# nvpro-samples/vk_gltf_renderer

Measured on AMD Instinct MI355X. Metric: Msamples/s (and ms/frame @ fixed spp) 1080p & 4K, 1/2/4/8 MI355X, higher is better.
Workload: dtype f32

## Files before the change

vk_gltf_renderer_amd/csrc/device/mi_pt_api.hip:

```cpp
#include <hip/hip_runtime.h>

#include <algorithm>
#include <chrono>
#include <cstdlib>
#include <cmath>
#include <cstdio>
#include <cstring>
#include <memory>
#include <string>
#include <vector>

#include "mi_pt.h"
#include "bvh_refit.h"
#include "material_patch.h"
#include "pt_build.h"
#include "pt_bvh.h"
#include "pt_deform.h"
#include "pt_kernels.h"

namespace {

thread_local std::string g_lastError;

int fail(int code, const std::string& msg)
// ... 248 lines not shown
  hipStream_t             lastStream = nullptr;
  hipStream_t             sideStream = nullptr;
  hipEvent_t              evShaded = nullptr, evShadowed = nullptr;

  ~MiPt()
  {
    if(bvhNodes)
      (void)hipFree(bvhNodes);
    if(bvhTris)
      (void)hipFree(bvhTris);
    if(bvh8Nodes)
      (void)hipFree(bvh8Nodes);
    for(hipEvent_t e : eventPool)
      (void)hipEventDestroy(e);
    for(hipEvent_t e : fcDone)
      if(e)
        (void)hipEventDestroy(e);
    if(fcHost)
      (void)hipHostFree(fcHost);
    if(sideStream)
      (void)hipStreamDestroy(sideStream);
    if(evShaded)
      (void)hipEventDestroy(evShaded);
    if(evShadowed)
      (void)hipEventDestroy(evShadowed);
  }
};

namespace {

size_t align16(size_t v) { return (v + 15u) & ~size_t(15); }

int allocPathResources(MiPt* pt, int frames)
{
  if(size_t(pt->numSlots) * size_t(frames) >= 0x7fffffffull)
    return fail(MI_PT_ERR_ARGUMENT, "too many path slots: reduce the frames in flight or the resolution");
  pt->framesCap          = frames;
  const size_t n         = std::max(size_t(pt->numSlots) * size_t(frames), size_t(1));
  HIP_TRY(pt->pathArrays.alloc(n));
  HIP_TRY(pt->firstHit.alloc(std::max(size_t(pt->numSlots), size_t(1))));
  pt->haveFirstHit = false;
  pt->optThroughput.release(); pt->optMisc.release(); pt->optMedium.release(); pt->optPixelSum.release(); pt->optGuides.release(); pt->optShadowAux2.release();
  pt::PathSoA& P = pt->paths;
  P              = pt::PathSoA{};
  P.radiance     = pt->pathArrays.ptr;
  P.firstHit     = pt->firstHit.ptr;
  const size_t numChunks = (n + pt::QCHUNK - 1) / pt::QCHUNK;
  const size_t subCap    = ((numChunks + pt::NSUB - 1) / pt::NSUB + 1) * pt::QCHUNK;
  const size_t qsize     = subCap * pt::NSUB;
  if(qsize >= (size_t(1) << 31))
    return fail(MI_PT_ERR_ARGUMENT, "mi_pt_render_frames: " + std::to_string(frames) + " frames in flight x " + std::to_string(pt->numSlots)
                                        + " pixel slots exceed 2^31 path slots");
  HIP_TRY(pt->queueMem.alloc(qsize * 3 + pt::QC_COUNT));
  HIP_TRY(pt->queuePayload.alloc(qsize * 14));
  pt->queueCap = qsize;
  pt::RayQueue* qs[3] = {&pt->queues.active[0], &pt->queues.active[1], &pt->queues.shadow};
  for(int i = 0; i < 3; ++i)
    qs[i]->slot = pt->queueMem.ptr + qsize * size_t(i);
  for(int i = 0; i < 2; ++i)
  {
    qs[i]->org  = pt->queuePayload.ptr + qsize * size_t(5 * i + 0);
    qs[i]->dir  = pt->queuePayload.ptr + qsize * size_t(5 * i + 1);
    qs[i]->aux2 = pt->queuePayload.ptr + qsize * size_t(5 * i + 2);
    qs[i]->misc = pt->queuePayload.ptr + qsize * size_t(5 * i + 3);
    qs[i]->rad  = pt->queuePayload.ptr + qsize * size_t(5 * i + 4);
    qs[i]->aux  = pt->queuePayload.ptr + qsize * 10;
  }
  pt->queues.shadow.org  = pt->queuePayload.ptr + qsize * 11;
  pt->queues.shadow.dir  = pt->queuePayload.ptr + qsize * 12;
  pt->queues.shadow.aux  = pt->queuePayload.ptr + qsize * 13;
  pt->queues.shadow.aux2 = nullptr;
  pt->queues.shadow.misc = pt->queues.shadow.rad = nullptr;
  pt->queues.counters = pt->queueMem.ptr + 3 * qsize;
  pt->queues.subCap   = uint32_t(subCap);
  pt->queues.candPool = nullptr; pt->queues.candNext = nullptr; pt->queues.overflow = nullptr;
  pt->queues.candCap  = 0;
  size_t candCap = qsize * 2;
  if(pt->sw.candPoolSet)
    candCap = pt->sw.candPool;
  if(pt->hasTransmissive && pt->wide && candCap > 0)
  {
    candCap = std::min(candCap, size_t(0x7fffffff));
    HIP_TRY(pt->candPool.alloc(candCap));
    HIP_TRY(pt->candLists.alloc(candCap + qsize));
    pt->queues.candPool = pt->candPool.ptr;
    pt->queues.candNext = pt->candLists.ptr;
    pt->queues.overflow = pt->candLists.ptr + candCap;
    pt->queues.candCap  = uint32_t(candCap);
  }
  HIP_TRY(hipMemset(pt->queues.counters, 0, sizeof(uint32_t) * pt::QC_COUNT));
  return MI_PT_OK;
}

int ensureOptionalPathArrays(MiPt* pt, bool stateBySlot, bool multiSample, bool guides, bool catcher)
{
  const size_t n = std::max(size_t(pt->numSlots) * size_t(pt->framesCap), size_t(1));
  auto need = [&](DevBuf<float4>& b, size_t count) -> int {
    if(b.ptr)
      return MI_PT_OK;
    HIP_TRY(hipDeviceSynchronize());
    HIP_TRY(b.alloc(count));
    HIP_TRY(hipMemset(b.ptr, 0, count * sizeof(float4)));
    return MI_PT_OK;
  };
  pt::PathSoA& P = pt->paths;
  if(stateBySlot || multiSample)
  {
    if(int rc = need(pt->optMisc, n)) return rc;
    P.misc = pt->optMisc.ptr;
  }
  if(stateBySlot)
  {
    if(int rc = need(pt->optThroughput, n)) return rc;
    P.throughput = pt->optThroughput.ptr;
  }
  if(multiSample)
  {
    if(int rc = need(pt->optPixelSum, n)) return rc;
    P.pixelSum = pt->optPixelSum.ptr;
  }
  if(!pt->simpleMaterials)
  {
    if(int rc = need(pt->optMedium, n)) return rc;
// ... 2020 lines not shown
```

vk_gltf_renderer_amd/csrc/device/pt_bvh.h:

```cpp
#pragma once
#include "pt_scene.h"

namespace pt {

#ifndef MI_BVH8_STACK_LDS
#define MI_BVH8_STACK_LDS 12
#endif
constexpr int BVH_STACK_LDS  = 2 * MI_BVH8_STACK_LDS;
constexpr int BVH_STACK_PRIV = 72;
constexpr int BVH_EMPTY      = int(0x80000000u);

struct TriHit
{
  float t, u, v;
  bool  front;
};

PT_DEV bool intersectTri(f3 v0, f3 e1, f3 e2, f3 org, f3 dir, TriHit& h)
{
#pragma clang fp contract(off)
  f3    pvec = crossFma(dir, e2);
  float det  = dotFma(e1, pvec);
  if(det == 0.0f)
    return false;
  float inv  = divExact(1.0f, det);
  f3    tvec = org - v0;
  float u    = dotFma(tvec, pvec) * inv;
  if(u < 0.0f || u > 1.0f)
    return false;
  f3    qvec = crossFma(tvec, e1);
  float v    = dotFma(dir, qvec) * inv;
  if(v < 0.0f || u + v > 1.0f)
    return false;
  h.t     = dotFma(e2, qvec) * inv;
  h.u     = u;
  h.v     = v;
  h.front = det > 0.0f;
  return true;
}

struct RaySetup
{
  f3 org, dir, idir, ood;
};
PT_DEV RaySetup makeRaySetup(f3 org, f3 dir)
{
  RaySetup    r;
  const float eps = 1e-30f;
  r.org           = org;
  r.dir           = dir;
  r.idir.x        = divExact(1.0f, fabsf(dir.x) < eps ? copysignf(eps, dir.x) : dir.x);
  r.idir.y        = divExact(1.0f, fabsf(dir.y) < eps ? copysignf(eps, dir.y) : dir.y);
  r.idir.z        = divExact(1.0f, fabsf(dir.z) < eps ? copysignf(eps, dir.z) : dir.z);
  r.ood           = org * r.idir;
  return r;
}

struct LaneStack
{
  int* lds;
  int  tid;
  int  stride;
  int* priv;
  int  sp;
  PT_DEV void push(int v)
  {
    if(sp < BVH_STACK_LDS)
      lds[sp * stride + tid] = v;
    else if(sp - BVH_STACK_LDS < BVH_STACK_PRIV)
      priv[sp - BVH_STACK_LDS] = v;
    ++sp;
  }
  PT_DEV int pop()
  {
    --sp;
    if(sp < BVH_STACK_LDS)
      return lds[sp * stride + tid];
    if(sp - BVH_STACK_LDS < BVH_STACK_PRIV)
      return priv[sp - BVH_STACK_LDS];
    return BVH_EMPTY;
  }
};

PT_DEV int bvhInnerStep(const DevScene& sc, const RaySetup& r, float tmax, int cur, LaneStack& st)
{
  const float4* n  = sc.bvhNodes + size_t(cur) * 4;
  const float4  n0 = n[0], n1 = n[1], n2 = n[2], n3 = n[3];
  float c0x0 = __fmaf_rn(n0.x, r.idir.x, -r.ood.x), c0x1 = __fmaf_rn(n0.y, r.idir.x, -r.ood.x);
  float c0y0 = __fmaf_rn(n0.z, r.idir.y, -r.ood.y), c0y1 = __fmaf_rn(n0.w, r.idir.y, -r.ood.y);
  float c0z0 = __fmaf_rn(n2.x, r.idir.z, -r.ood.z), c0z1 = __fmaf_rn(n2.y, r.idir.z, -r.ood.z);
  float c1x0 = __fmaf_rn(n1.x, r.idir.x, -r.ood.x), c1x1 = __fmaf_rn(n1.y, r.idir.x, -r.ood.x);
  float c1y0 = __fmaf_rn(n1.z, r.idir.y, -r.ood.y), c1y1 = __fmaf_rn(n1.w, r.idir.y, -r.ood.y);
  float c1z0 = __fmaf_rn(n2.z, r.idir.z, -r.ood.z), c1z1 = __fmaf_rn(n2.w, r.idir.z, -r.ood.z);
  float t0n  = fmaxf(fmaxf(fminf(c0x0, c0x1), fminf(c0y0, c0y1)), fmaxf(fminf(c0z0, c0z1), 0.0f));
  float t0f  = fminf(fminf(fmaxf(c0x0, c0x1), fmaxf(c0y0, c0y1)), fminf(fmaxf(c0z0, c0z1), tmax));
  float t1n  = fmaxf(fmaxf(fminf(c1x0, c1x1), fminf(c1y0, c1y1)), fmaxf(fminf(c1z0, c1z1), 0.0f));
  float t1f  = fminf(fminf(fmaxf(c1x0, c1x1), fmaxf(c1y0, c1y1)), fminf(fmaxf(c1z0, c1z1), tmax));
  bool  hit0 = t0n <= t0f * 1.0000012f + 1e-30f;
  bool  hit1 = t1n <= t1f * 1.0000012f + 1e-30f;
  int   ch0 = __float_as_int(n3.x), ch1 = __float_as_int(n3.y);
  if(hit0 && hit1)
  {
    bool swap = t1n < t0n;
    st.push(swap ? ch0 : ch1);
    return swap ? ch1 : ch0;
  }
  if(hit0)
    return ch0;
  if(hit1)
// ... 26 lines not shown
```

vk_gltf_renderer_amd/csrc/device/pt_kernels.hip:

```cpp
#include <hip/hip_runtime.h>
#include <hip/hip_fp16.h>

#ifndef MI_PT_EXACT_FP
#define PT_FAST_SHADING_MATH 1
#endif
#include "pt_kernels.h"
#include "pt_shading.h"
#include "pt_bvh.h"
#include "pt_bvh8.h"
#include "pt_packet.h"
#include "pt_feed.h"
#include "pt_visualize.h"

namespace pt {

namespace {

constexpr int TRACE_BLOCK = 1024;
#ifndef NODE_CACHE_EXTRA
#define NODE_CACHE_EXTRA 0
#endif
constexpr int NODE_CACHE  = 712 + NODE_CACHE_EXTRA;
constexpr int NODE_CACHE_ALPHA = 504 + NODE_CACHE_EXTRA;
constexpr int SEL_BLOCK   = 256;
// ... 258 lines not shown
__device__ __noinline__ f4 missEnvironmentCall(const DevScene& scIn, const FrameConsts& fcIn, f3 rayDir, float lastSamplePdf)
{
  const DevScene&    sc = uniformConst(scIn);
  const FrameConsts& fc = uniformConst(fcIn);
  float envPdf;
  f3    envColor;
  sampleEnvironment(sc, fc, rayDir, envColor, envPdf);
  return mk4(envColor.x, envColor.y, envColor.z, computeEnvHitMisWeight(sc, fc, lastSamplePdf, envPdf));
}
PT_DEV void missEnvironment(const DevScene& sc, const FrameConsts& fc, f3 rayDir, float lastSamplePdf, f3& envColor, float& mis)
{
  const f4 r = missEnvironmentCall(sc, fc, rayDir, lastSamplePdf);
  envColor   = xyz(r);
  mis        = r.w;
}
PT_DEV float infinitePlaneT(const FrameConsts& fc, f3 rayOrigin, f3 rayDir, float hitT)
{
  if(!hasFlag(fc.frameInfo.flags, MI_SCENE_USE_INFINITE_PLANE))
    return -1.0f;
  const float planeHeight = fc.frameInfo.infinitePlaneDistance, Dn = rayDir.y;
  if(rayOrigin.y > planeHeight && fabsf(Dn) > 1e-6f)
  {
    const float t = divExact(-rayOrigin.y + planeHeight, Dn);
    if(t > 0.0f && t < hitT)
      return t;
  }
  return -1.0f;
}

__global__ void __launch_bounds__(256) k_generate(DevScene sc, FrameConsts fc, PathSoA P, Queues Q, const uint32_t* ownedTiles, int sampleIndex,
                                                   StatCounters* stats)
{
  const uint32_t batchSlots = uint32_t(fc.numSlots) * uint32_t(fc.numFrames);
  uint32_t       slot       = blockIdx.x * blockDim.x + threadIdx.x;
  CameraPath     cp{};
  if(slot < batchSlots)
    cp = generateCameraPath(fc, P, ownedTiles, slot, sampleIndex);
  if(cp.valid)
  {
    if(P.misc)
      P.misc[slot] = make_float4(0.0f, __uint_as_float(PF_ALIVE), __uint_as_float(cp.seed), 0.0f);
    if(stats)
      atomicAdd(&stats->cameraPaths, 1ull);
  }
  if(slot < batchSlots)
  {
    const uint32_t chunk = slot / QCHUNK;
    const uint32_t pos   = (chunk % NSUB) * Q.subCap + (chunk / NSUB) * QCHUNK + (slot % QCHUNK);
    Q.active[0].slot[pos] = cp.valid ? slot : QUEUE_DEAD;
    if(cp.valid)
    {
      Q.active[0].org[pos] = make_float4(cp.origin.x, cp.origin.y, cp.origin.z, 0.0f);
      Q.active[0].dir[pos] = make_float4(cp.direction.x, cp.direction.y, cp.direction.z, __uint_as_float(cp.seed));
      if(fc.stateInQueue)
        Q.active[0].misc[pos] = make_float4(0.0f, __uint_as_float(PF_ALIVE), __uint_as_float(cp.seed), 0.0f);
    }
  }
  if(blockIdx.x == 0 && threadIdx.x < NSUB)
  {
    const uint32_t numChunks = batchSlots / QCHUNK;
    Q.counters[QC_PAIR0 + 2 * threadIdx.x] = QCHUNK * (numChunks / NSUB + (threadIdx.x < numChunks % NSUB ? 1u : 0u));
  }
  if(blockIdx.x == 0 && threadIdx.x < 8)
    Q.counters[QC_HEADS_TRACE + threadIdx.x] = 0;
  (void)sc;
}

#ifdef TRACE_PROFILE
__device__ unsigned long long g_traceProf[20];
__device__ unsigned long long g_shadowProf[16];
#define PROF_T() __builtin_amdgcn_s_memtime()
#define PROF_ADD(i, t0) profAcc[i] += PROF_T() - (t0)
#define PROF_CNT(i, n) profCnt[i] += (unsigned long long)(n)
#else
#define PROF_T() 0ull
#define PROF_ADD(i, t0) (void)(t0)
#define PROF_CNT(i, n) (void)0
#endif

#ifdef SHADE_PROFILE
__device__ unsigned long long g_shadeProf[20];
#define SPROF_BEGIN() const unsigned long long sprofT0_ = __builtin_amdgcn_s_memtime(); const int sprofLanes_ = __popcll(__ballot(true))
#define SPROF_END(r)                                                                                                             \
  do                                                                                                                             \
  {                                                                                                                              \
    if(!FIRST)                                                                                                                   \
    {                                                                                                                            \
      const unsigned long long dt_ = __builtin_amdgcn_s_memtime() - sprofT0_;                                                   \
      if(laneId() == uint32_t(__ffsll((long long)__ballot(true)) - 1))                                                          \
      {                                                                                                                          \
        atomicAdd(&g_shadeProf[2 * (r)], dt_);                                                                                   \
        atomicAdd(&g_shadeProf[2 * (r) + 1], dt_ * (unsigned long long)sprofLanes_);                                             \
      }                                                                                                                          \
    }                                                                                                                            \
  } while(0)
#else
#define SPROF_BEGIN() (void)0
#define SPROF_END(r) (void)0
#endif

#ifndef REFILL_IDLE_LANES
#define REFILL_IDLE_LANES 16
#endif
#ifndef TRI_PHASE_LANES_N
#define TRI_PHASE_LANES_N 24
#endif
constexpr int TRI_PHASE_LANES      = TRI_PHASE_LANES_N;
constexpr int TRI_PHASE_EXIT_LANES = 10;
#ifndef TRI_ROUND_LANES
#define TRI_ROUND_LANES 20
#endif
#ifndef TRI_ROUND_LANE_CAP_N
#define TRI_ROUND_LANE_CAP_N 4
#endif
constexpr int TRI_ROUND_LANE_CAP = TRI_ROUND_LANE_CAP_N;
#ifndef ALPHA_ROUND_MIN
#define ALPHA_ROUND_MIN 32
#endif
#ifndef ALPHA_ROUND_WAITING
#define ALPHA_ROUND_WAITING 8
#endif

PT_DEV uint32_t fillNodeCache(const DevScene& sc, uint4* s_nodes, uint32_t capacity = NODE_CACHE)
{
  const uint32_t n = min(uint32_t(sc.bvh8NumNodes), capacity);
  for(uint32_t i = threadIdx.x; i < n * 5u; i += blockDim.x)
    s_nodes[i] = sc.bvh8Nodes[i];
  __syncthreads();
  return n;
}

struct ClosestBest
{
  float    t, u, v;
  int      tri;
  uint32_t rnode, prim;
};
template <bool HAS_ALPHA>
PT_DEV void closestTestLoaded(const DevScene& sc, const RaySetup& r, const DevTri& T, int triIndex, ClosestBest& best, uint32_t& seed0, bool& seedLoaded,
                              const float4* misc, uint32_t slot);
template <bool HAS_ALPHA>
PT_DEV void closestTestTriangle(const DevScene& sc, const RaySetup& r, int triIndex, ClosestBest& best, uint32_t& seed0, bool& seedLoaded,
                                const float4* misc, uint32_t slot)
{
  const DevTri T = sc.tris[triIndex];
  closestTestLoaded<HAS_ALPHA>(sc, r, T, triIndex, best, seed0, seedLoaded, misc, slot);
}
template <bool HAS_ALPHA>
PT_DEV void closestTestLoaded(const DevScene& sc, const RaySetup& r, const DevTri& T, int triIndex, ClosestBest& best, uint32_t& seed0, bool& seedLoaded,
                              const float4* misc, uint32_t slot)
{
  TriHit       h;
  if(!intersectTri(xyz(T.a), xyz(T.b), xyz(T.c), r.org, r.dir, h) || !(h.t > 0.0f))
    return;
  const uint32_t rnode = __float_as_uint(T.a.w), prim = __float_as_uint(T.b.w), flags = __float_as_uint(T.c.w);
// ... 279 lines not shown
    if(__ballot(needAlpha) & mine)
      aPending = true;
  }
  if(__ballot(commits) & mine)
    occluded = true;
}

template <bool WIDE, bool HAS_ALPHA, bool COUNT>
__global__ void __launch_bounds__(TRACE_BLOCK, TRACE_MIN_WAVES) k_trace_closest(DevScene sc, PathSoA P, Queues Q, int cur, StatCounters* stats)
{
  __shared__ int      s_stack[BVH_STACK_LDS * TRACE_BLOCK];
  __shared__ uint32_t s_prefix[NSUB + 1];
  constexpr int CACHE = HAS_ALPHA ? NODE_CACHE_ALPHA : NODE_CACHE;
  __shared__ uint4    s_nodes[WIDE ? CACHE * 5 : 1];
  __shared__ unsigned long long s_slots[WIDE ? TRACE_BLOCK : 1];
  __shared__ uint4    s_alpha[(WIDE && HAS_ALPHA) ? TRACE_BLOCK : 1];

  static_assert(2 * BVH8_STACK_LDS == BVH_STACK_LDS, "both stack flavours share one LDS allocation");
  if(blockIdx.x == 0 && threadIdx.x < NSUB)
  {
    Q.counters[(cur ? QC_PAIR0 : QC_PAIR1) + 2 * threadIdx.x]     = 0;
    Q.counters[(cur ? QC_PAIR0 : QC_PAIR1) + 2 * threadIdx.x + 1] = 0;
  }
  const RayQueue in = Q.active[cur];
  queuePrefix(&Q.counters[cur ? QC_PAIR1 : QC_PAIR0], s_prefix);
  WaveFeed feed;
  feedInit(feed, s_prefix[NSUB]);
  if(!feedBlockHasWork(feed))
    return;
  const uint32_t cachedNodes = WIDE ? fillNodeCache(sc, s_nodes, uint32_t(CACHE)) : 0u;
  LaneStack  st;
  LaneStack2 st2;
  int        stackOverflow[WIDE ? 2 * BVH8_STACK_PRIV : BVH_STACK_PRIV];
  st.lds = s_stack;  st.tid = int(threadIdx.x);  st.stride = TRACE_BLOCK;  st.sp = 0;  st.priv = stackOverflow;
  st2.lds = s_stack; st2.tid = int(threadIdx.x); st2.stride = TRACE_BLOCK; st2.sp = 0;
  st2.privBase = reinterpret_cast<uint32_t*>(stackOverflow); st2.privBits = reinterpret_cast<uint32_t*>(stackOverflow) + (WIDE ? BVH8_STACK_PRIV : 0);
  bool        active = false;
  uint32_t    slot = 0, pos = 0;
  RaySetup    r{};
  int         node = BVH_EMPTY;
  NodeGroup   G{0, 0};
  uint32_t    octinv = 0;
  uint32_t    pBase = 0, pMask = 0, qBase = 0, qMask = 0;
  int         lastVisiting = 64;
  uint32_t    aCount   = 0;
  bool        aPending = false;
  uint4*      waveAlpha = s_alpha + ((WIDE && HAS_ALPHA) ? (threadIdx.x & ~63u) : 0u);
  ClosestBest best{INFINITE_F, 0.0f, 0.0f, -1, 0xffffffffu, 0xffffffffu};
  uint32_t    seed0 = 0;
  bool        seedLoaded = false;
  unsigned    nodes = 0, tris = 0, rays = 0;
  bool     pValid = false;
  uint32_t pPos = 0, pSlot = QUEUE_DEAD;
  float4   pO = make_float4(0, 0, 0, 0), pD = make_float4(0, 0, 0, 0);
#ifdef TRACE_PROFILE
  unsigned long long profAcc[10] = {0, 0, 0, 0, 0, 0, 0, 0, 0, 0};
  unsigned long long profCnt[10] = {0, 0, 0, 0, 0, 0, 0, 0, 0, 0};
  const unsigned long long profStart = PROF_T();
#endif
  for(;;)
  {
    const unsigned long long tFeed = PROF_T();
    PROF_CNT(4, 1);
    PROF_CNT(5, 64 - __popcll(__ballot(active)));
    if(!active && pValid)
    {
      pValid = false;
      if(pSlot != QUEUE_DEAD)
      {
        slot       = pSlot;
        pos        = pPos;
        r          = makeRaySetup(xyz(pO), xyz(pD));
        best       = ClosestBest{INFINITE_F, 0.0f, 0.0f, -1, 0xffffffffu, 0xffffffffu};
        seed0      = __float_as_uint(pD.w);
        seedLoaded = true;
        if(WIDE)
        {
          octinv = rayOctInv(r.idir);
          G      = rootGroup(octinv);
          st2.sp = 0;
        }
        else
        {
          st.sp = 0;
          node  = sc.bvhRoot;
        }
        active = sc.bvhRoot != BVH_EMPTY;
        if(!active)
          in.aux[pos] = make_float4(INFINITE_F, __int_as_float(-1), 0.0f, 0.0f);
        if(COUNT) ++rays;
      }
    }
    PROF_ADD(4, tFeed);
    if(!feed.exhausted)
    {
      const unsigned long long tTake = PROF_T();
      uint32_t flat = feedTake(feed, !pValid, &Q.counters[QC_HEADS_TRACE]);
      PROF_ADD(5, tTake);
      const unsigned long long tIssue = PROF_T();
      if(flat != 0xffffffffu)
      {
        pPos   = queuePos(Q.subCap, s_prefix, flat);
        pSlot  = in.slot[pPos];
        pO     = in.org[pPos];
        pD     = in.dir[pPos];
        pValid = true;
      }
      PROF_ADD(6, tIssue);
    }
    const bool moreWork = !feed.exhausted || __ballot(pValid) != 0ull;
    if(__ballot(active) == 0ull)
    {
      if(!moreWork)
        break;
      continue;
    }
    PROF_ADD(0, tFeed);
    for(;;)
    {
      if(WIDE)
      {
        const auto nodeStep = [&]() -> bool {
          const unsigned long long tNode = PROF_T();
          bool visited = false;
          if(active && !leafPending(qMask))
          {
            if((G.bits >> 8) == 0u && st2.sp > 0)
              G = st2.pop();
            if(G.bits >> 8)
            {
              const uint32_t child = groupPopChild(G, octinv);
              if(G.bits >> 8)
                st2.push(G);
              uint32_t tBase, tMask;
              bvh8Visit(sc, r, best.t, octinv, child, G, tBase, tMask, s_nodes, cachedNodes);
              if(COUNT) ++nodes;
              visited = true;
              if(leafPending(tMask))
              {
                if(!leafPending(pMask)) { pBase = tBase; pMask = tMask; }
                else                    { qBase = tBase; qMask = tMask; }
              }
            }
          }
          PROF_ADD(1, tNode);
          return visited;
        };
        bool               visited = false;
        unsigned long long pend    = __ballot(active && leafPending(pMask));
        const bool         drain   = lastVisiting < TRI_PHASE_LANES;
        if(pend != 0ull && (drain || __popcll(pend) >= TRI_ROUND_LANES))
        {
          const unsigned long long tTri0 = PROF_T();
          TriRound           tr;
          PROF_CNT(2, 1);
          PROF_CNT(3, __popcll(pend));
          triRoundPublish<true>(sc, active, pBase, pMask, qBase, qMask, reinterpret_cast<uint32_t*>(s_slots + (threadIdx.x & ~63u)), tr);
          PROF_ADD(2, tTri0);
// ... 5 lines not shown
          triRoundFinish<HAS_ALPHA, COUNT>(sc, r, best, seed0, tr, tris, s_slots + (threadIdx.x & ~63u), waveAlpha, aCount, aPending);
#endif
          PROF_ADD(2, tFinish);
        }
        else
          visited = nodeStep();
        PROF_CNT(0, 1);
        PROF_CNT(1, __popcll(__ballot(visited)));
        PROF_CNT(7, __popcll(__ballot(active && leafPending(qMask))));
        lastVisiting = __popcll(__ballot(visited));
        const unsigned long long tTri = PROF_T();
        if(HAS_ALPHA && aCount != 0u)
        {
          const bool walked  = active && !leafPending(pMask) && (G.bits >> 8) == 0u && st2.sp == 0;
          const int  waiting = __popcll(__ballot(walked && aPending));
          if(aCount >= ALPHA_ROUND_MIN || lastVisiting < TRI_PHASE_LANES || waiting >= ALPHA_ROUND_WAITING)
          {
            const unsigned long long tAlpha = PROF_T();
            bool none = false;
            alphaRound<false>(sc, seed0, waveAlpha, aCount, aPending, best, none);
            PROF_ADD(8, tAlpha);
            PROF_CNT(8, 1);
          }
        }
        PROF_ADD(2, tTri);
        if(active && !leafPending(pMask) && (G.bits >> 8) == 0u && st2.sp == 0 && !(HAS_ALPHA && aPending))
        {
          in.aux[pos] = make_float4(best.t, __int_as_float(best.tri), best.u, best.v);
          active      = false;
        }
      }
      else if(active)
      {
        bool finished = false;
#pragma unroll 1
        for(int k = 0; k < 4 && node >= 0; ++k)
        {
          node = bvhInnerStep(sc, r, best.t, node, st);
          if(COUNT) ++nodes;
        }
        if(node < 0 && node != BVH_EMPTY)
        {
          if(COUNT) ++tris;
          closestTestTriangle<HAS_ALPHA>(sc, r, ~node, best, seed0, seedLoaded, P.misc, slot);
          node = bvhPop(st);
        }
        finished = node == BVH_EMPTY;
        if(finished)
        {
          in.aux[pos] = make_float4(best.t, __int_as_float(best.tri), best.u, best.v);
          active      = false;
        }
      }
      const unsigned long long act = __ballot(active);
      if(act == 0ull || (moreWork && __popcll(act) <= 64 - REFILL_IDLE_LANES))
        break;
    }
  }
#ifdef TRACE_PROFILE
  if(laneId() == 0)
  {
    atomicAdd(&g_traceProf[0], profAcc[0]);
    atomicAdd(&g_traceProf[1], profAcc[1]);
    atomicAdd(&g_traceProf[2], profAcc[2]);
    atomicAdd(&g_traceProf[3], PROF_T() - profStart);
    atomicAdd(&g_traceProf[4], 1ull);
    atomicAdd(&g_traceProf[5], profAcc[4]);
    atomicAdd(&g_traceProf[6], profAcc[5]);
    atomicAdd(&g_traceProf[7], profAcc[6]);
    for(int i = 0; i < 8; ++i)
      atomicAdd(&g_traceProf[8 + i], profCnt[i]);
    atomicAdd(&g_traceProf[16], profAcc[3]);
    atomicAdd(&g_traceProf[17], profAcc[7]);
    atomicAdd(&g_traceProf[18], profAcc[8]);
    atomicAdd(&g_traceProf[19], profCnt[8]);
  }
#endif
  if(COUNT)
  {
    atomicAdd(&stats->segments, (unsigned long long)rays);
    atomicAdd(&stats->nodesClosest, (unsigned long long)nodes);
    atomicAdd(&stats->trisClosest, (unsigned long long)tris);
  }
}

constexpr int PACKET_STACK = 96;

typedef uint32_t u32x4s __attribute__((ext_vector_type(4)));
PT_DEV void scalarLoadNode(const uint4* nodes, uint32_t index, uint4& n0, uint4& n1, uint4& n2, uint4& n3, uint4& n4)
{
  const uint64_t addr = uint64_t(reinterpret_cast<uintptr_t>(nodes)) + uint64_t(index) * 80ull;
  const uint64_t A    = (uint64_t(uint32_t(__builtin_amdgcn_readfirstlane(uint32_t(addr >> 32)))) << 32) | uint64_t(uint32_t(__builtin_amdgcn_readfirstlane(uint32_t(addr))));
  u32x4s         a, b, c, d, e;
  asm volatile("s_load_dwordx4 %0, %5, 0x0\n\ts_load_dwordx4 %1, %5, 0x10\n\ts_load_dwordx4 %2, %5, 0x20\n\ts_load_dwordx4 %3, %5, 0x30\n\t"
               "s_load_dwordx4 %4, %5, 0x40\n\ts_waitcnt lgkmcnt(0)"
               : "=&s"(a), "=&s"(b), "=&s"(c), "=&s"(d), "=&s"(e)
               : "s"(A)
               : "memory");
  n0 = make_uint4(a[0], a[1], a[2], a[3]); n1 = make_uint4(b[0], b[1], b[2], b[3]); n2 = make_uint4(c[0], c[1], c[2], c[3]);
  n3 = make_uint4(d[0], d[1], d[2], d[3]); n4 = make_uint4(e[0], e[1], e[2], e[3]);
}
PT_DEV void scalarLoadNodePlanes(const uint4* nodes, const float* planes, uint32_t index, uint32_t offNx, uint32_t offNy, uint32_t offNz, uint32_t offFx,
                                 uint32_t offFy, uint32_t offFz, uint4& n0, uint4& n1, f32x8s& pnx, f32x8s& pny, f32x8s& pnz, f32x8s& pfx, f32x8s& pfy,
                                 f32x8s& pfz)
{
  const uint64_t addr = uint64_t(reinterpret_cast<uintptr_t>(nodes)) + uint64_t(index) * 80ull;
  const uint64_t A    = (uint64_t(uint32_t(__builtin_amdgcn_readfirstlane(uint32_t(addr >> 32)))) << 32) | uint64_t(uint32_t(__builtin_amdgcn_readfirstlane(uint32_t(addr))));
  const uint64_t pad  = uint64_t(reinterpret_cast<uintptr_t>(planes)) + uint64_t(index) * 192ull;
  const uint64_t Pn   = (uint64_t(uint32_t(__builtin_amdgcn_readfirstlane(uint32_t(pad >> 32)))) << 32) | uint64_t(uint32_t(__builtin_amdgcn_readfirstlane(uint32_t(pad))));
// ... 415 lines not shown

template <bool WIDE, int MODE, bool COUNT>
__global__ void __launch_bounds__(ShadowCfg<MODE>::BLOCK, TRACE_MIN_WAVES) k_trace_shadow(DevScene sc, const DevScene* __restrict__ scp, PathSoA P, Queues Q, int nxt, float catcherDarken, StatCounters* stats, int overflowOnly)
{
  constexpr int  SBLOCK    = ShadowCfg<MODE>::BLOCK;
  constexpr bool HAS_ALPHA = MODE >= 1, HAS_TRANS = MODE == 2, REC = MODE == 3;
  constexpr bool DEFER = MODE == 1 || MODE == 3;
  static_assert(!REC || WIDE, "the recording walk exists for the 8-wide BVH only");
  __shared__ int      s_stack[BVH_STACK_LDS * SBLOCK];
  __shared__ uint32_t s_prefix[NSUB + 1];
  __shared__ uint4    s_nodes[WIDE ? ShadowCfg<MODE>::CACHE * 5 : 1];
  __shared__ uint32_t s_items[(WIDE && !HAS_TRANS) ? SBLOCK : 1];
  __shared__ uint4    s_alpha[(WIDE && DEFER) ? SBLOCK : 1];
  __shared__ uint32_t s_head[REC ? SBLOCK : 1], s_ovf[REC ? SBLOCK : 1];
  __shared__ uint8_t  s_octLut[(WIDE && MI_PT_OCT_LUT) ? OCT_LUT_BYTES : 1];
  queuePrefix(&Q.counters[(nxt ? QC_PAIR1 : QC_PAIR0) + 1], s_prefix);
  const RayQueue in = Q.shadow;
  const bool     subset = MODE == 2 && overflowOnly != 0;
  uint32_t* const heads = &Q.counters[subset ? QC_HEADS_OVERFLOW : QC_HEADS_SHADOW];
  WaveFeed feed;
  feedInit(feed, subset ? Q.counters[QC_OVERFLOW] : s_prefix[NSUB]);
  if(!feedBlockHasWork(feed))
    return;
  if(WIDE && MI_PT_OCT_LUT)
    fillOctLut(s_octLut);
  const uint32_t cachedNodes = WIDE ? fillNodeCache(sc, s_nodes, uint32_t(ShadowCfg<MODE>::CACHE)) : 0u;
  LaneStack  st;
  LaneStack2 st2;
  int        stackOverflow[WIDE ? 2 * BVH8_STACK_PRIV : BVH_STACK_PRIV];
  st.lds = s_stack;  st.tid = int(threadIdx.x);  st.stride = SBLOCK;  st.sp = 0;  st.priv = stackOverflow;
  st2.lds = s_stack; st2.tid = int(threadIdx.x); st2.stride = SBLOCK; st2.sp = 0;
  st2.privBase = reinterpret_cast<uint32_t*>(stackOverflow); st2.privBits = reinterpret_cast<uint32_t*>(stackOverflow) + (WIDE ? BVH8_STACK_PRIV : 0);
  bool      active = false;
  uint32_t  slot   = 0;
  RaySetup  r{};
  int       node = BVH_EMPTY;
  NodeGroup G{0, 0};
  uint32_t  octinv = 0;
  float     tMax  = 0.0f;
  int       phase = 0;
  unsigned  nTrans = 0;
  bool      occluded = false;
  uint32_t  seed0 = 0;
  f3        contrib = mk3(0.0f);
  float    bT = 0.0f, bU = 0.0f, bV = 0.0f, lastT = -1.0f, prevHitT = 0.0f;
  uint32_t bRnode = 0, bPrim = 0, lastRnode = 0, lastPrim = 0;
  int      bTri = 0;
  bool     found = false, haveLast = false, isInside = false;
  f3       total = mk3(1.0f);
  unsigned nodes = 0, tris = 0, rays = 0;
  bool     pValid = false;
  uint32_t pSlot = QUEUE_DEAD, pQPos = 0, qpos = 0;
  float4   pO = make_float4(0, 0, 0, 0), pD = make_float4(0, 0, 0, 0), pC = make_float4(0, 0, 0, 0);
  bool     catcherRay = false;
  uint32_t pBase = 0, pMask = 0, qBase = 0, qMask = 0;
  uint32_t aCount   = 0;
  bool     aPending = false;
  bool     toOverflow = false;
#ifdef TRACE_PROFILE
  unsigned long long sp[16] = {0, 0, 0, 0, 0, 0, 0, 0, 0, 0, 0, 0, 0, 0, 0, 0};
  const unsigned long long spStart = PROF_T();
#define SPROF_ADD(i, t0) sp[i] += PROF_T() - (t0)
#define SPROF_CNT(i, n) sp[i] += (unsigned long long)(n)
#else
#define SPROF_ADD(i, t0) (void)(t0)
#define SPROF_CNT(i, n) (void)0
#endif
  uint4*   waveAlpha = s_alpha + ((WIDE && DEFER) ? (threadIdx.x & ~63u) : 0u);
  CandRec  rec{Q.candPool, Q.candNext, &Q.counters[QC_CAND_POOL], Q.candCap, s_head + (REC ? (threadIdx.x & ~63u) : 0u), s_ovf + (REC ? (threadIdx.x & ~63u) : 0u), 0u, 0u};
  (void)rec;

  auto deposit = [&](bool occ) { shadowDeposit(P, Q, nxt, slot, qpos, catcherRay, contrib, total, occ, catcherDarken); };

  constexpr unsigned SHADOW_CANDS = 8;
  float    cT[HAS_TRANS ? SHADOW_CANDS : 1], cU[HAS_TRANS ? SHADOW_CANDS : 1], cV[HAS_TRANS ? SHADOW_CANDS : 1];
  uint32_t cR[HAS_TRANS ? SHADOW_CANDS : 1], cP[HAS_TRANS ? SHADOW_CANDS : 1];
  int      cI[HAS_TRANS ? SHADOW_CANDS : 1];
  auto processCandidate = [&](float t, int tri, uint32_t rnode, uint32_t prim, float u, float v) {
    f3    bary    = mk3(1.0f - u - v, u, v);
    float opacity = getOpacityFast(sc, tri, bary);
    if(candidateRand(seed0, int(rnode), int(prim)) < opacity)
    {
      float segment = fmaxf(0.0f, t - prevHitT);
      f3    curT    = getShadowTransmission(*scp, int(rnode), int(prim), bary, segment, r.dir, isInside);
      prevHitT      = t;
      total *= curT;
      if(maxComp(total) <= MIN_TRANSMISSION)
        occluded = true;
    }
  };

  auto restartWalk = [&]() {
    if(WIDE)
    {
      G      = rootGroup(octinv);
      st2.sp = 0;
      pMask = qMask = 0u;
    }
    else
    {
      st.sp = 0;
      node  = sc.bvhRoot;
    }
  };
  auto testTriLoaded = [&](const DevTri& T, int triIndex) {
    if(COUNT) ++tris;
    const uint32_t flags = __float_as_uint(T.c.w);
    TriHit         h;
    const bool consider = !HAS_TRANS || phase == 0 || ((flags & INST_TRANSMISSIVE) && !(flags & INST_FORCE_OPAQUE));
    if(!(consider && intersectTri(xyz(T.a), xyz(T.b), xyz(T.c), r.org, r.dir, h) && h.t > 0.0f && h.t < tMax))
      return;
    const uint32_t rnode = __float_as_uint(T.a.w), prim = __float_as_uint(T.b.w);
    if(!HAS_TRANS || phase == 0)
    {
      if(!HAS_ALPHA || (flags & INST_FORCE_OPAQUE))
        occluded = true;
      else if(HAS_TRANS && (flags & INST_TRANSMISSIVE))
      {
        if(nTrans < SHADOW_CANDS)
        {
          cT[nTrans] = h.t; cI[nTrans] = triIndex; cR[nTrans] = rnode; cP[nTrans] = prim; cU[nTrans] = h.u; cV[nTrans] = h.v;
        }
        ++nTrans;
      }
      else
      {
        float opacity = getOpacityFast(sc, triIndex, mk3(1.0f - h.u - h.v, h.u, h.v));
        if(candidateRand(seed0, int(rnode), int(prim)) < opacity)
          occluded = true;
      }
    }
    else
    {
      const bool afterLast  = !haveLast || h.t > lastT || (h.t == lastT && (rnode > lastRnode || (rnode == lastRnode && prim > lastPrim)));
      const bool beforeBest = !found || h.t < bT || (h.t == bT && (rnode < bRnode || (rnode == bRnode && prim < bPrim)));
      if(afterLast && beforeBest)
      {
        found = true; bT = h.t; bTri = triIndex; bRnode = rnode; bPrim = prim; bU = h.u; bV = h.v;
      }
    }
  };

  auto testTri = [&](int triIndex) { testTriLoaded(sc.tris[triIndex], triIndex); };

  for(;;)
  {
    const unsigned long long tOuter = PROF_T();
    SPROF_CNT(8, 1);
    SPROF_CNT(9, 64 - __popcll(__ballot(active)));
    if(!active && pValid)
    {
      pValid = false;
      if(pSlot != QUEUE_DEAD)
      {
        slot     = pSlot;
        qpos     = pQPos;
        r        = makeRaySetup(xyz(pO), xyz(pD));
        tMax     = pO.w;
        isInside = (__float_as_uint(pD.w) & 1u) != 0u;
        catcherRay = (__float_as_uint(pD.w) & 2u) != 0u;
        contrib  = xyz(pC);
        seed0    = __float_as_uint(pC.w);
        phase    = 0;
        nTrans   = 0;
        occluded = false;
        total    = mk3(1.0f);
        haveLast = false;
        found    = false;
        prevHitT = 0.0f;
        octinv   = rayOctInv(r.idir) ^ (MODE == 2 ? 0u : sc.shadowOctFlip);
        restartWalk();
        active = true;
        if(REC)
        {
          s_head[threadIdx.x] = CAND_NIL;
          s_ovf[threadIdx.x]  = 0u;
        }
        if(COUNT) ++rays;
        if(sc.bvhRoot == BVH_EMPTY)
        {
          if(HAS_TRANS)
            deposit(false);
          else
            reinterpret_cast<uint32_t*>(&Q.shadow.org[qpos])[3] = CAND_NIL;
          active = false;
        }
      }
    }
    if(!feed.exhausted)
    {
      uint32_t flat = feedTake(feed, !pValid, heads);
      if(flat != 0xffffffffu)
      {
        const uint32_t pPos = subset ? Q.overflow[flat] : queuePos(Q.subCap, s_prefix, flat);
        pQPos  = pPos;
        pSlot  = in.slot[pPos];
        pO     = in.org[pPos];
        pD     = in.dir[pPos];
        pC     = in.aux[pPos];
        pValid = true;
      }
    }
    const bool moreWork = !feed.exhausted || __ballot(pValid) != 0ull;
    SPROF_ADD(0, tOuter);
    if(__ballot(active) == 0ull)
    {
      if(!moreWork)
        break;
      continue;
    }
    for(;;)
    {
      bool walkDone = false;
      const unsigned long long tInner = PROF_T();
      SPROF_CNT(10, 1);
      SPROF_CNT(11, __popcll(__ballot(active)));
      if(WIDE)
      {
        bool visited = false;
        if(active && !leafPending(qMask) && !(DEFER && occluded))
        {
          const float walkTmax = (HAS_TRANS && phase == 1 && found) ? bT : tMax;
          if((G.bits >> 8) == 0u && st2.sp > 0)
            G = st2.pop();
          if(G.bits >> 8)
          {
            const uint32_t child = groupPopChild(G, octinv);
            if(G.bits >> 8)
              st2.push(G);
            uint32_t tBase, tMask;
            bvh8Visit(sc, r, walkTmax, octinv, child, G, tBase, tMask, s_nodes, cachedNodes, s_octLut);
            if(COUNT) ++nodes;
            visited = true;
            if(leafPending(tMask))
            {
              if(!leafPending(pMask)) { pBase = tBase; pMask = tMask; }
              else                    { qBase = tBase; qMask = tMask; }
            }
          }
        }
        SPROF_ADD(1, tInner);
        SPROF_CNT(12, __popcll(__ballot(visited)));
        const unsigned long long tTri = PROF_T();
        unsigned long long pend = __ballot(active && leafPending(pMask));
        if(!HAS_TRANS)
        {
          if(pend != 0ull)
          {
            const int  visiting = __popcll(__ballot(visited));
            const bool drain    = visiting < TRI_PHASE_LANES;
            if(drain || __popcll(pend) >= TRI_ROUND_LANES)
            {
// ... 94 lines not shown
          if(HAS_TRANS && !occluded && !(phase == 1 && !found))
          {
            if(phase == 1)
            {
              haveLast = true; lastT = bT; lastRnode = bRnode; lastPrim = bPrim;
              processCandidate(bT, bTri, bRnode, bPrim, bU, bV);
              --nTrans;
            }
            if(!occluded && nTrans > 0)
            {
              phase = 1;
              found = false;
              restartWalk();
              finished = false;
            }
          }
          if(finished)
          {
            if(HAS_TRANS)
              deposit(occluded);
            else
            {
              uint32_t code = occluded ? SHADOW_OCCLUDED : CAND_NIL;
              if(REC && !occluded)
              {
                code       = s_head[threadIdx.x];
                toOverflow = s_ovf[threadIdx.x] != 0u;
              }
              if(toOverflow)
                reinterpret_cast<uint32_t*>(&Q.shadow.dir[qpos])[3] |= SHADOW_DIR_OVERFLOW;
              else
                reinterpret_cast<uint32_t*>(&Q.shadow.org[qpos])[3] = code;
            }
            active = false;
          }
        }
      }
      if(REC)
      {
        const unsigned long long mO = __ballot(toOverflow);
        if(mO != 0ull)
        {
          const int first = __ffsll((long long)mO) - 1;
          uint32_t  base  = 0u;
          if(int(laneId()) == first)
            base = atomicAdd(&Q.counters[QC_OVERFLOW], uint32_t(__popcll(mO)));
          base = uint32_t(__builtin_amdgcn_readlane(int(base), first));
          if(toOverflow)
            Q.overflow[base + laneCountBelow(mO)] = qpos;
        }
        toOverflow = false;
      }
      SPROF_ADD(4, tFin);
      const unsigned long long act = __ballot(active);
      if(act == 0ull || (moreWork && __popcll(act) <= 64 - REFILL_IDLE_LANES))
        break;
    }
  }
#ifdef TRACE_PROFILE
  if(laneId() == 0 && WIDE && DEFER)
  {
    sp[5] = PROF_T() - spStart;
    sp[6] = 1;
    for(int i = 0; i < 16; ++i)
      atomicAdd(&g_shadowProf[i], sp[i]);
  }
#endif
#undef SPROF_ADD
#undef SPROF_CNT
  if(COUNT)
  {
    atomicAdd(&stats->shadowRays, (unsigned long long)rays);
    atomicAdd(&stats->nodesShadow, (unsigned long long)nodes);
    atomicAdd(&stats->trisShadow, (unsigned long long)tris);
  }
}

PT_DEV void resolveChain(const DevScene& sc, const PathSoA& P, const Queues& Q, int nxt, uint32_t qpos, uint32_t slot, float4 d4, float4 c4, uint32_t code, bool catcherRay,
                         float catcherDarken)
{
  f3             total    = mk3(1.0f);
  bool           occluded = false;
  const f3       dir      = xyz(d4);
  const uint32_t seed0    = __float_as_uint(c4.w);
  bool           isInside = (__float_as_uint(d4.w) & 1u) != 0u, haveLast = false;
  float          lastT = -1.0f, prevHitT = 0.0f;
  uint32_t       lastRnode = 0u, lastPrim = 0u;
  for(;;)
  {
    uint32_t best = CAND_NIL, bRnode = 0u, bPrim = 0u;
    bool     bIds = false;
    float4   bC   = make_float4(0, 0, 0, 0);
    for(uint32_t k = code; k != CAND_NIL; k = Q.candNext[k])
    {
      const float4   c   = Q.candPool[k];
      const uint32_t tri = __float_as_uint(c.w);
      const bool     tieLast = haveLast && c.x == lastT, tieBest = best != CAND_NIL && c.x == bC.x;
      uint32_t       rnode = 0u, prim = 0u;
      if(tieLast || tieBest)
      {
        rnode = __float_as_uint(gat(sc.tris, tri).a.w);
        prim  = __float_as_uint(gat(sc.tris, tri).b.w);
      }
      const bool afterLast  = !haveLast || c.x > lastT || (tieLast && (rnode > lastRnode || (rnode == lastRnode && prim > lastPrim)));
      bool       beforeBest = best == CAND_NIL || c.x < bC.x;
      if(tieBest)
      {
        if(!bIds)
        {
// ... 523 lines not shown
```

vk_gltf_renderer_amd/csrc/device/pt_scene.h:

```cpp
#pragma once
#include <hip/hip_runtime.h>
#include <stdint.h>

#include "mi_pt.h"
#include "pt_math.h"

namespace pt {

struct DevTexture
{
  uint32_t levelOffset[16];
  uint16_t width, height;
  uint8_t  numLevels;
  uint8_t  srgb;
  uint8_t  magFilter, minFilter, mipmapMode, wrapS, wrapT;
  uint8_t  _pad[5];
};

struct DevTexRef
{
  float    uv[6];
  uint32_t level0;
  uint16_t width, height;
  uint8_t  numLevels, srgb, magFilter, minFilter, mipmapMode, wrapS, wrapT, texCoord;
// ... 193 lines not shown
    return pixelSlot * uint32_t(fc.numFrames) + frame;
  return ((pixelSlot >> 6) * uint32_t(fc.numFrames) + frame) * 64u + (pixelSlot & 63u);
}
__device__ __forceinline__ uint32_t pathSlotFrame(const FrameConsts& fc, uint32_t slot)
{
  if(fc.numFrames <= 1)
    return 0u;
  const uint32_t w = fc.slotLayout == 1 ? slot : (slot >> 6), q = __umulhi(w, fc.framesMagic) >> fc.framesShift;
  return w - q * uint32_t(fc.numFrames);
}
__device__ __forceinline__ uint32_t pathSlotPixel(const FrameConsts& fc, uint32_t slot)
{
  if(fc.numFrames <= 1)
    return slot;
  const uint32_t w = fc.slotLayout == 1 ? slot : (slot >> 6), q = __umulhi(w, fc.framesMagic) >> fc.framesShift;
  return fc.slotLayout == 1 ? q : (q * 64u + (slot & 63u));
}
#endif

enum : uint32_t
{
  PF_INSIDE     = 1u << 0,
  PF_NOT_SOLID  = 1u << 1,
  PF_ALIVE      = 1u << 2,
  PF_PLANE_HIT  = 1u << 3,
  PF_PRIMARY_MISS = 1u << 4,
  PF_DEPTH_SHIFT   = 8,
  PF_SCATTER_SHIFT = 16,
};
constexpr uint32_t RADW_NOT_SOLID    = 0x80000000u;
constexpr uint32_t RADW_PRIMARY_MISS = 0xffc00001u;

struct PathSoA
{
  float4*   radiance;
  float4*   firstHit;
  float4*   misc;
  float4*   throughput;
  uint4*    medium;
  float4*   pixelSum;
  float4*   guideAlbedo;
  float4*   guideNormal;
};

constexpr int      NSUB       = 16;
constexpr int      QCHUNK     = 256;
constexpr uint32_t QUEUE_DEAD = 0xffffffffu;
struct RayQueue
{
  uint32_t* slot;
  float4*   org;
  float4*   dir;
  float4*   aux;
  float4*   aux2;
  float4*   misc;
  float4*   rad;
};
constexpr uint32_t SHADOW_TARGET_QUEUE = 0x80000000u;
struct Queues
{
  RayQueue  active[2];
  RayQueue  shadow;
  uint32_t* counters;
  uint32_t  subCap;
  float4*   candPool;
  uint32_t* candNext;
  uint32_t* overflow;
  uint32_t  candCap;
};
constexpr uint32_t CAND_NIL        = 0xffffffffu;
constexpr uint32_t SHADOW_OCCLUDED = 0xfffffffeu;
constexpr uint32_t SHADOW_DIR_OVERFLOW = 4u;
enum : int
{
  QC_PAIR0        = 0,
  QC_PAIR1        = 32,
  QC_HEADS_TRACE  = 96,
  QC_HEADS_SHADOW = 128,
  QC_HEADS_OVERFLOW = 160,
  QC_CAND_POOL      = 192,
  QC_RESOLVE        = 224,
  QC_OVERFLOW       = 256,
  QC_COUNT          = 288
};

struct StatCounters
{
  unsigned long long cameraPaths, segments, shadowRays, nodesClosest, trisClosest, nodesShadow, trisShadow, textureTaps, surfaceHits, nodesPrimary, trisPrimary;
};

}
```

vk_gltf_renderer_amd/csrc/device/pt_shade_body.h:

```cpp
  const DevScene&    sc = uniformConst(*scp);
  const FrameConsts& fc = uniformConst(*fcp);
  const bool         stateInQueue = fc.stateInQueue != 0;
  __shared__ uint32_t s_prefix[NSUB + 1];
  __shared__ uint32_t s_push[4];
  __shared__ float    s_srgb[256];
#ifndef SHADE_NO_DEFERRED_MISS
  constexpr bool DEFER_MISS = !FIRST;
#else
  constexpr bool DEFER_MISS = false;
#endif
  __shared__ uint32_t s_missPos[DEFER_MISS ? 2 * SHADE_BLOCK : 1];
  __shared__ uint32_t s_missCount;
  const bool          deferMiss = DEFER_MISS && !hasFlag(fc.frameInfo.flags, MI_SCENE_USE_INFINITE_PLANE) && !hasFlag(fc.frameInfo.flags, MI_SCENE_USE_HDR_ENVIRONMENT);
  if(threadIdx.x == 0)
    s_missCount = 0;
  auto finishMisses = [&](bool all) {
    __syncthreads();
    const uint32_t n = s_missCount;
    if(n == 0u || (!all && n < uint32_t(SHADE_BLOCK)))
      return;
    const uint32_t take = min(n, uint32_t(SHADE_BLOCK)), base = n - take;
    uint32_t       pos = 0;
    if(threadIdx.x < take)
      pos = s_missPos[base + threadIdx.x];
// ... 488 lines not shown
                done = true;
              else
                throughput /= rrPcont;
            }
            if(!done)
            {
              surfaceDepth++;
              rayDir = normalize(rayDir);
            }
          }
        }
        (void)earlyContinue;
      }

      if(FIRST && P.guideAlbedo && !guideWritten && fc.pc.numSamples == 1)
      {
        P.guideAlbedo[slot] = make_float4(0, 0, 0, 0);
        P.guideNormal[slot] = make_float4(0, 0, 0, 0);
      }
      alive = !done && surfaceDepth < maxDepth;
      flags = (isInside ? PF_INSIDE : 0u) | (solid ? 0u : PF_NOT_SOLID) | (alive ? PF_ALIVE : 0u) | (uint32_t(min(surfaceDepth, 255)) << PF_DEPTH_SHIFT)
              | (uint32_t(scatterBounces) << PF_SCATTER_SHIFT);
      nextRad  = make_float4(radiance.x, radiance.y, radiance.z, __uint_as_float(__float_as_uint(fmaxf(maxRoughness.x, 0.0f)) | (solid ? 0u : RADW_NOT_SOLID)));
      nextMisc = make_float4(maxRoughness.y, __uint_as_float(flags), __uint_as_float(seed), coneWidth);
      if((!stateInQueue || !alive) && !deferred)
      {
        P.radiance[slot] = nextRad;
        if(P.misc)
          P.misc[slot] = nextMisc;
      }
      if(alive)
      {
        nextOrg = make_float4(rayOrigin.x, rayOrigin.y, rayOrigin.z, 0.0f);
        nextDir = make_float4(rayDir.x, rayDir.y, rayDir.z, __uint_as_float(seed));
        nextThr = make_float4(throughput.x, throughput.y, throughput.z, lastSamplePdf);
        if(!stateInQueue)
          P.throughput[slot] = nextThr;
      }
      if(COUNT && taps)
        atomicAdd(&stats->textureTaps, (unsigned long long)taps);
      if(COUNT && (meshHit || hitInfinitePlane))
        atomicAdd(&stats->surfaceHits, 1ull);
    }
#ifdef SHADE_PROFILE
    const unsigned long long sprofPush0 = __builtin_amdgcn_s_memtime();
#endif
    const PushPos  pp      = queuePushBlock2(alive, pushShadow, Q.subCap, &Q.counters[(nxt ? QC_PAIR1 : QC_PAIR0) + 2 * (chunk % NSUB)], chunk % NSUB, s_push);
    const uint32_t posNext = pp.next, posShadow = pp.shadow;
    if(alive)
    {
      Q.active[nxt].slot[posNext] = slot;
      Q.active[nxt].org[posNext]  = nextOrg;
      Q.active[nxt].dir[posNext]  = nextDir;
      if(stateInQueue)
      {
        Q.active[nxt].rad[posNext]  = nextRad;
        Q.active[nxt].misc[posNext] = nextMisc;
        Q.active[nxt].aux2[posNext] = nextThr;
      }
    }
    if(pushShadow)
    {
      Q.shadow.slot[posShadow] = (stateInQueue && alive) ? (posNext | SHADOW_TARGET_QUEUE) : slot;
      Q.shadow.org[posShadow]  = shOrg;
      Q.shadow.dir[posShadow]  = shDir;
      Q.shadow.aux[posShadow]  = shCon;
      if(catcher)
        Q.shadow.aux2[posShadow] = make_float4(shCon2.x, shCon2.y, shCon2.z, __uint_as_float(alive ? posNext : 0xffffffffu));
    }
#ifdef SHADE_PROFILE
    if(!FIRST && laneId() == 0)
    {
      const unsigned long long t_ = __builtin_amdgcn_s_memtime();
      atomicAdd(&g_shadeProf[14], t_ - sprofPush0);
      atomicAdd(&g_shadeProf[15], (t_ - sprofPush0) * (unsigned long long)__popcll(__ballot(alive || pushShadow)));
    }
    const unsigned long long sprofFin0 = __builtin_amdgcn_s_memtime();
#endif
    if(DEFER_MISS && deferMiss)
      finishMisses(false);
#ifdef SHADE_PROFILE
    if(!FIRST && laneId() == 0)
    {
      const unsigned long long t_ = __builtin_amdgcn_s_memtime();
      atomicAdd(&g_shadeProf[16], t_ - sprofFin0);
      atomicAdd(&g_shadeProf[18], t_ - sprofRound0);
      atomicAdd(&g_shadeProf[19], (t_ - sprofRound0) * (unsigned long long)__popcll(__ballot(inRange && slot != QUEUE_DEAD)));
    }
#endif
   }
   if(CAN_SORT)
     __syncthreads();
  }
  if(DEFER_MISS && deferMiss)
  {
    finishMisses(true);
    finishMisses(true);
  }
```

Before: 750.2.

## Precompute ray reciprocals in queues and restart idle lanes inside the wide trace loop

The shade and camera kernels now compute each ray's inverse direction and store it in the queue payload: in the previously shared aux slot for active queues, and in a new inv array for shadow rays. The wide trace and shadow kernels load this instead of doing three exact divisions per ray. The wide kernels also restart rays on idle lanes inside the inner traversal loop once enough lanes are startable, and leave to fetch more work only when enough lanes lack a prefetched ray. The aim is to cut divergence and idle-lane cost in traversal, at the price of more queue memory traffic, a larger payload allocation, and a shadow contrib load skipped when there is no transmission.

```diff
diff --git a/vk_gltf_renderer_amd/csrc/device/mi_pt_api.hip b/vk_gltf_renderer_amd/csrc/device/mi_pt_api.hip
--- a/vk_gltf_renderer_amd/csrc/device/mi_pt_api.hip
+++ b/vk_gltf_renderer_amd/csrc/device/mi_pt_api.hip
@@ -324,7 +324,7 @@
     return fail(MI_PT_ERR_ARGUMENT, "mi_pt_render_frames: " + std::to_string(frames) + " frames in flight x " + std::to_string(pt->numSlots)
                                         + " pixel slots exceed 2^31 path slots");
   HIP_TRY(pt->queueMem.alloc(qsize * 3 + pt::QC_COUNT));
-  HIP_TRY(pt->queuePayload.alloc(qsize * 14));
+  HIP_TRY(pt->queuePayload.alloc(qsize * 16));
   pt->queueCap = qsize;
   pt::RayQueue* qs[3] = {&pt->queues.active[0], &pt->queues.active[1], &pt->queues.shadow};
   for(int i = 0; i < 3; ++i)
@@ -336,11 +336,13 @@
     qs[i]->aux2 = pt->queuePayload.ptr + qsize * size_t(5 * i + 2);
     qs[i]->misc = pt->queuePayload.ptr + qsize * size_t(5 * i + 3);
     qs[i]->rad  = pt->queuePayload.ptr + qsize * size_t(5 * i + 4);
-    qs[i]->aux  = pt->queuePayload.ptr + qsize * 10;
-  }
-  pt->queues.shadow.org  = pt->queuePayload.ptr + qsize * 11;
-  pt->queues.shadow.dir  = pt->queuePayload.ptr + qsize * 12;
-  pt->queues.shadow.aux  = pt->queuePayload.ptr + qsize * 13;
+    qs[i]->aux  = pt->queuePayload.ptr + qsize * size_t(10 + i);
+    qs[i]->inv  = nullptr;
+  }
+  pt->queues.shadow.org  = pt->queuePayload.ptr + qsize * 12;
+  pt->queues.shadow.dir  = pt->queuePayload.ptr + qsize * 13;
+  pt->queues.shadow.aux  = pt->queuePayload.ptr + qsize * 14;
+  pt->queues.shadow.inv  = pt->queuePayload.ptr + qsize * 15;
   pt->queues.shadow.aux2 = nullptr;
   pt->queues.shadow.misc = pt->queues.shadow.rad = nullptr;
   pt->queues.counters = pt->queueMem.ptr + 3 * qsize;
diff --git a/vk_gltf_renderer_amd/csrc/device/pt_bvh.h b/vk_gltf_renderer_amd/csrc/device/pt_bvh.h
--- a/vk_gltf_renderer_amd/csrc/device/pt_bvh.h
+++ b/vk_gltf_renderer_amd/csrc/device/pt_bvh.h
@@ -43,18 +43,25 @@
 {
   f3 org, dir, idir, ood;
 };
-PT_DEV RaySetup makeRaySetup(f3 org, f3 dir)
+PT_DEV f3 rayReciprocal(f3 dir)
 {
-  RaySetup    r;
   const float eps = 1e-30f;
-  r.org           = org;
-  r.dir           = dir;
-  r.idir.x        = divExact(1.0f, fabsf(dir.x) < eps ? copysignf(eps, dir.x) : dir.x);
-  r.idir.y        = divExact(1.0f, fabsf(dir.y) < eps ? copysignf(eps, dir.y) : dir.y);
-  r.idir.z        = divExact(1.0f, fabsf(dir.z) < eps ? copysignf(eps, dir.z) : dir.z);
-  r.ood           = org * r.idir;
+  f3          idir;
+  idir.x = divExact(1.0f, fabsf(dir.x) < eps ? copysignf(eps, dir.x) : dir.x);
+  idir.y = divExact(1.0f, fabsf(dir.y) < eps ? copysignf(eps, dir.y) : dir.y);
+  idir.z = divExact(1.0f, fabsf(dir.z) < eps ? copysignf(eps, dir.z) : dir.z);
+  return idir;
+}
+PT_DEV RaySetup loadedRaySetup(f3 org, f3 dir, f3 idir)
+{
+  RaySetup r;
+  r.org  = org;
+  r.dir  = dir;
+  r.idir = idir;
+  r.ood  = org * idir;
   return r;
 }
+PT_DEV RaySetup makeRaySetup(f3 org, f3 dir) { return loadedRaySetup(org, dir, rayReciprocal(dir)); }
 
 struct LaneStack
 {
diff --git a/vk_gltf_renderer_amd/csrc/device/pt_kernels.hip b/vk_gltf_renderer_amd/csrc/device/pt_kernels.hip
--- a/vk_gltf_renderer_amd/csrc/device/pt_kernels.hip
+++ b/vk_gltf_renderer_amd/csrc/device/pt_kernels.hip
@@ -334,6 +334,8 @@
     {
       Q.active[0].org[pos] = make_float4(cp.origin.x, cp.origin.y, cp.origin.z, 0.0f);
       Q.active[0].dir[pos] = make_float4(cp.direction.x, cp.direction.y, cp.direction.z, __uint_as_float(cp.seed));
+      const f3 inv         = rayReciprocal(cp.direction);
+      Q.active[0].aux[pos] = make_float4(inv.x, inv.y, inv.z, 0.0f);
       if(fc.stateInQueue)
         Q.active[0].misc[pos] = make_float4(0.0f, __uint_as_float(PF_ALIVE), __uint_as_float(cp.seed), 0.0f);
     }
@@ -383,6 +385,12 @@
 
 #ifndef REFILL_IDLE_LANES
 #define REFILL_IDLE_LANES 16
+#endif
+#ifndef START_LANES
+#define START_LANES 4
+#endif
+#ifndef FETCH_LANES
+#define FETCH_LANES 16
 #endif
 #ifndef TRI_PHASE_LANES_N
 #define TRI_PHASE_LANES_N 24
@@ -768,17 +776,13 @@
   unsigned    nodes = 0, tris = 0, rays = 0;
   bool     pValid = false;
   uint32_t pPos = 0, pSlot = QUEUE_DEAD;
-  float4   pO = make_float4(0, 0, 0, 0), pD = make_float4(0, 0, 0, 0);
+  float4   pO = make_float4(0, 0, 0, 0), pD = make_float4(0, 0, 0, 0), pI = make_float4(0, 0, 0, 0);
 #ifdef TRACE_PROFILE
   unsigned long long profAcc[10] = {0, 0, 0, 0, 0, 0, 0, 0, 0, 0};
   unsigned long long profCnt[10] = {0, 0, 0, 0, 0, 0, 0, 0, 0, 0};
   const unsigned long long profStart = PROF_T();
 #endif
-  for(;;)
-  {
-    const unsigned long long tFeed = PROF_T();
-    PROF_CNT(4, 1);
-    PROF_CNT(5, 64 - __popcll(__ballot(active)));
+  const auto startRay = [&]() {
     if(!active && pValid)
     {
       pValid = false;
@@ -786,7 +790,7 @@
       {
         slot       = pSlot;
         pos        = pPos;
-        r          = makeRaySetup(xyz(pO), xyz(pD));
+        r          = WIDE ? loadedRaySetup(xyz(pO), xyz(pD), xyz(pI)) : makeRaySetup(xyz(pO), xyz(pD));
         best       = ClosestBest{INFINITE_F, 0.0f, 0.0f, -1, 0xffffffffu, 0xffffffffu};
         seed0      = __float_as_uint(pD.w);
         seedLoaded = true;
@@ -807,6 +811,13 @@
         if(COUNT) ++rays;
       }
     }
+  };
+  for(;;)
+  {
+    const unsigned long long tFeed = PROF_T();
+    PROF_CNT(4, 1);
+    PROF_CNT(5, 64 - __popcll(__ballot(active)));
+    startRay();
     PROF_ADD(4, tFeed);
     if(!feed.exhausted)
     {
@@ -820,6 +831,8 @@
         pSlot  = in.slot[pPos];
         pO     = in.org[pPos];
         pD     = in.dir[pPos];
+        if(WIDE)
+          pI = in.aux[pPos];
         pValid = true;
       }
       PROF_ADD(6, tIssue);
@@ -931,9 +944,24 @@
           active      = false;
         }
       }
-      const unsigned long long act = __ballot(active);
-      if(act == 0ull || (moreWork && __popcll(act) <= 64 - REFILL_IDLE_LANES))
-        break;
+      if(WIDE)
+      {
+        const unsigned long long startable = __ballot(!active && pValid);
+        if(startable != 0ull && (__popcll(startable) >= START_LANES || __ballot(active) == 0ull))
+        {
+          const unsigned long long tStart = PROF_T();
+          startRay();
+          PROF_ADD(4, tStart);
+        }
+        if(__ballot(active) == 0ull || (!feed.exhausted && __popcll(__ballot(!pValid)) >= FETCH_LANES))
+          break;
+      }
+      else
+      {
+        const unsigned long long act = __ballot(active);
+        if(act == 0ull || (moreWork && __popcll(act) <= 64 - REFILL_IDLE_LANES))
+          break;
+      }
     }
   }
 #ifdef TRACE_PROFILE
@@ -1455,6 +1483,8 @@
   bool     pValid = false;
   uint32_t pSlot = QUEUE_DEAD, pQPos = 0, qpos = 0;
   float4   pO = make_float4(0, 0, 0, 0), pD = make_float4(0, 0, 0, 0), pC = make_float4(0, 0, 0, 0);
+  float4   pI = make_float4(0, 0, 0, 0);
+  constexpr bool NEED_AUX = !WIDE || HAS_TRANS;
   bool     catcherRay = false;
   uint32_t pBase = 0, pMask = 0, qBase = 0, qMask = 0;
   uint32_t aCount   = 0;
@@ -1546,11 +1576,7 @@
 
   auto testTri = [&](int triIndex) { testTriLoaded(sc.tris[triIndex], triIndex); };
 
-  for(;;)
-  {
-    const unsigned long long tOuter = PROF_T();
-    SPROF_CNT(8, 1);
-    SPROF_CNT(9, 64 - __popcll(__ballot(active)));
+  const auto startRay = [&]() {
     if(!active && pValid)
     {
       pValid = false;
@@ -1558,12 +1584,13 @@
       {
         slot     = pSlot;
         qpos     = pQPos;
-        r        = makeRaySetup(xyz(pO), xyz(pD));
+        r        = WIDE ? loadedRaySetup(xyz(pO), xyz(pD), xyz(pI)) : makeRaySetup(xyz(pO), xyz(pD));
         tMax     = pO.w;
         isInside = (__float_as_uint(pD.w) & 1u) != 0u;
         catcherRay = (__float_as_uint(pD.w) & 2u) != 0u;
-        contrib  = xyz(pC);
-        seed0    = __float_as_uint(pC.w);
+        if(NEED_AUX)
+          contrib = xyz(pC);
+        seed0    = __float_as_uint(WIDE ? pI.w : pC.w);
         phase    = 0;
         nTrans   = 0;
         occluded = false;
@@ -1590,6 +1617,13 @@
         }
       }
     }
+  };
+  for(;;)
+  {
+    const unsigned long long tOuter = PROF_T();
+    SPROF_CNT(8, 1);
+    SPROF_CNT(9, 64 - __popcll(__ballot(active)));
+    startRay();
     if(!feed.exhausted)
     {
       uint32_t flat = feedTake(feed, !pValid, heads);
@@ -1600,7 +1634,10 @@
         pSlot  = in.slot[pPos];
         pO     = in.org[pPos];
         pD     = in.dir[pPos];
-        pC     = in.aux[pPos];
+        if(WIDE)
+          pI = in.inv[pPos];
+        if(NEED_AUX)
+          pC = in.aux[pPos];
         pValid = true;
       }
     }
@@ -1801,9 +1838,24 @@
         toOverflow = false;
       }
       SPROF_ADD(4, tFin);
-      const unsigned long long act = __ballot(active);
-      if(act == 0ull || (moreWork && __popcll(act) <= 64 - REFILL_IDLE_LANES))
-        break;
+      if(WIDE)
+      {
+        const unsigned long long startable = __ballot(!active && pValid);
+        if(startable != 0ull && (__popcll(startable) >= START_LANES || __ballot(active) == 0ull))
+        {
+          const unsigned long long tStart = PROF_T();
+          startRay();
+          SPROF_ADD(0, tStart);
+        }
+        if(__ballot(active) == 0ull || (!feed.exhausted && __popcll(__ballot(!pValid)) >= FETCH_LANES))
+          break;
+      }
+      else
+      {
+        const unsigned long long act = __ballot(active);
+        if(act == 0ull || (moreWork && __popcll(act) <= 64 - REFILL_IDLE_LANES))
+          break;
+      }
     }
   }
 #ifdef TRACE_PROFILE
diff --git a/vk_gltf_renderer_amd/csrc/device/pt_scene.h b/vk_gltf_renderer_amd/csrc/device/pt_scene.h
--- a/vk_gltf_renderer_amd/csrc/device/pt_scene.h
+++ b/vk_gltf_renderer_amd/csrc/device/pt_scene.h
@@ -269,6 +269,7 @@
   float4*   org;
   float4*   dir;
   float4*   aux;
+  float4*   inv;
   float4*   aux2;
   float4*   misc;
   float4*   rad;
diff --git a/vk_gltf_renderer_amd/csrc/device/pt_shade_body.h b/vk_gltf_renderer_amd/csrc/device/pt_shade_body.h
--- a/vk_gltf_renderer_amd/csrc/device/pt_shade_body.h
+++ b/vk_gltf_renderer_amd/csrc/device/pt_shade_body.h
@@ -564,6 +564,8 @@
       Q.active[nxt].slot[posNext] = slot;
       Q.active[nxt].org[posNext]  = nextOrg;
       Q.active[nxt].dir[posNext]  = nextDir;
+      const f3 nextInv = rayReciprocal(xyz(nextDir));
+      Q.active[nxt].aux[posNext]  = make_float4(nextInv.x, nextInv.y, nextInv.z, 0.0f);
       if(stateInQueue)
       {
         Q.active[nxt].rad[posNext]  = nextRad;
@@ -577,6 +579,8 @@
       Q.shadow.org[posShadow]  = shOrg;
       Q.shadow.dir[posShadow]  = shDir;
       Q.shadow.aux[posShadow]  = shCon;
+      const f3 shInv = rayReciprocal(xyz(shDir));
+      Q.shadow.inv[posShadow]  = make_float4(shInv.x, shInv.y, shInv.z, shCon.w);
       if(catcher)
         Q.shadow.aux2[posShadow] = make_float4(shCon2.x, shCon2.y, shCon2.z, __uint_as_float(alive ? posNext : 0xffffffffu));
     }
```

Measured after the change: 732.6. 0.976x the previous value.
